# JunyiPeng00/wespeaker_hubert

Measured on AMD Instinct MI355X. Metric: embeddings/sec on 5s 16kHz utts, higher is better.
Workload: dtype f32 (bf16x3 split MFMA, fp32 accumulate)

## Files before the change

wespeaker_hubert_amd/csrc/astp_fused.h:

```cpp
#pragma once

#include "common.h"

namespace wsp {

struct AstpArgs {
  const float* att;
  const float* x;
  int ldx, B, T, C;
  const int* seg;
  const void* w2;
  const float* bias2;
  float var_floor;
  float* out;
};
bool astp_fused_supported(int C, int K);
void launch_astp_fused(const AstpArgs& p, hipStream_t s);

}
```

wespeaker_hubert_amd/csrc/astp_fused.hip:

```cpp
#include "astp_fused.h"
#include "gemm_common.h"

namespace wsp {

namespace {

typedef __bf16 bf16x8 __attribute__((ext_vector_type(8)));

constexpr int kK = 128;

typedef __attribute__((address_space(3))) void lds_void;

__device__ __forceinline__ void dma16(__amdgpu_buffer_rsrc_t r, unsigned char* lds, int voff) {
  __builtin_amdgcn_raw_ptr_buffer_load_lds(r, (lds_void*)lds, 16, voff, 0, 0, 0);
}

constexpr int kCB2 = 256;
constexpr int kChunkBytes = 32 * kK * 4;

constexpr int kLds3 = 3 * kChunkBytes;

__global__ __launch_bounds__(512, 1) void astp_fused3_kernel(const AstpArgs p) {
  extern __shared__ __attribute__((aligned(16))) unsigned char ring[];
  const int tid = threadIdx.x;
  const int lane = tid & 63;
  const int wave = tid >> 6;
  const int r32 = lane & 31;
  const int h = lane >> 5;
  const int nct = p.C / kCB2;
  const int id = xcd_remap(blockIdx.x, gridDim.x);
  const int b = id / nct;
  const int ct = id - b * nct;
  const int r0 = p.seg ? p.seg[b] : b * p.T;
  const int T = p.seg ? p.seg[b + 1] - r0 : p.T;
  const int col = ct * kCB2 + wave * 32 + r32;
  const __amdgpu_buffer_rsrc_t ra = make_rsrc(p.att + (size_t)r0 * kK);
  const __amdgpu_buffer_rsrc_t rx = make_rsrc(p.x + (size_t)r0 * p.ldx);

  auto dma_chunk = [&](int t0, int slot) {
#pragma unroll
    for (int j = 0; j < 2; ++j) {
      const int piece = 2 * wave + j;
      const int row = 2 * piece + h;
      const int c = r32 ^ (row & 15);
      const int t = t0 + row;
      dma16(ra, ring + slot * kChunkBytes + piece * 1024, t < T ? (t * kK + c * 4) * 4 : kOOB);
    }
  };
  auto load_x = [&](int t0, float (&xv)[16]) {
#pragma unroll
    for (int r = 0; r < 16; ++r) {
      const int t = t0 + (r & 3) + 8 * (r >> 2) + 4 * h;
      xv[r] = __builtin_bit_cast(float, __builtin_amdgcn_raw_buffer_load_b32(
                                            rx, t < T ? (t * p.ldx + col) * 4 : kOOB, 0, 0));
    }
  };
  bf16x8 wf[16];
  {
    const __amdgpu_buffer_rsrc_t rw = make_rsrc(p.w2);
    const int ntile = p.C / 32;
#pragma unroll
    for (int i = 0; i < 16; ++i)
      wf[i] = __builtin_bit_cast(bf16x8, __builtin_amdgcn_raw_buffer_load_b128(
                                             rw, ((i * ntile + ct * (kCB2 / 32) + wave) * 64 + lane) * 16, 0, 0));
  }
  const float bias = p.bias2[col];

  float m = -INFINITY, s = 0.f, a1 = 0.f, a2 = 0.f;
  auto consume = [&](int t0, int slot, const float (&xv)[16]) {
    const unsigned char* ab = ring + slot * kChunkBytes + r32 * 512;
    f32x16 acc;
#pragma unroll
    for (int r = 0; r < 16; ++r) acc[r] = 0.f;
#pragma unroll
    for (int ks = 0; ks < 8; ++ks) {
      const int c0 = 4 * ks + 2 * h;
      const f32x4 v0 = *reinterpret_cast<const f32x4*>(ab + ((c0 ^ (r32 & 15)) << 4));
      const f32x4 v1 = *reinterpret_cast<const f32x4*>(ab + (((c0 + 1) ^ (r32 & 15)) << 4));
      bf16x8 ah, al;
#pragma unroll
      for (int e = 0; e < 8; ++e) {
        const float v = e < 4 ? v0[e] : v1[e - 4];
        const __bf16 hh = (__bf16)v;
        ah[e] = hh;
        al[e] = (__bf16)(v - (float)hh);
      }
      acc = __builtin_amdgcn_mfma_f32_32x32x16_bf16(al, wf[2 * ks], acc, 0, 0, 0);
      acc = __builtin_amdgcn_mfma_f32_32x32x16_bf16(ah, wf[2 * ks + 1], acc, 0, 0, 0);
      acc = __builtin_amdgcn_mfma_f32_32x32x16_bf16(ah, wf[2 * ks], acc, 0, 0, 0);
    }
    float ev[16], mc = -INFINITY;
#pragma unroll
    for (int r = 0; r < 16; ++r) {
      const int t = t0 + (r & 3) + 8 * (r >> 2) + 4 * h;
      ev[r] = t < T ? acc[r] + bias : -INFINITY;
      mc = fmaxf(mc, ev[r]);
    }
    if (mc != -INFINITY) {
      const float m1 = fmaxf(m, mc);
      const float sc = __expf(m - m1);
      s *= sc;
      a1 *= sc;
      a2 *= sc;
#pragma unroll
      for (int r = 0; r < 16; ++r) {
        const float pe = __expf(ev[r] - m1);
        s += pe;
        a1 = fmaf(pe, xv[r], a1);
        a2 = fmaf(pe * xv[r], xv[r], a2);
      }
      m = m1;
    }
  };

  float xa[16], xb[16], xc[16];
  const int nch = (T + 31) / 32;
  dma_chunk(0, 0);
  load_x(0, xa);
  if (nch > 1) {
    dma_chunk(32, 1);
    load_x(32, xb);
  }
  auto step = [&](int c, int slot, const float (&xcur)[16], float (&xnext2)[16]) {
    if (c + 1 < nch)
      asm volatile("s_waitcnt vmcnt(18)" ::: "memory");
    else
      asm volatile("s_waitcnt vmcnt(0)" ::: "memory");
    __syncthreads();
    if (c + 2 < nch) {
      dma_chunk((c + 2) * 32, slot == 0 ? 2 : slot - 1);
      load_x((c + 2) * 32, xnext2);
    }
    consume(c * 32, slot, xcur);
  };
  for (int c = 0; c < nch; c += 3) {
    step(c, 0, xa, xc);
    if (c + 1 >= nch) break;
    step(c + 1, 1, xb, xa);
    if (c + 2 >= nch) break;
    step(c + 2, 2, xc, xb);
  }
  const float mo = __shfl_xor(m, 32), so = __shfl_xor(s, 32), a1o = __shfl_xor(a1, 32), a2o = __shfl_xor(a2, 32);
  const float M = fmaxf(m, mo);
  const float f0 = m == -INFINITY ? 0.f : __expf(m - M);
  const float f1 = mo == -INFINITY ? 0.f : __expf(mo - M);
  const float S = s * f0 + so * f1;
  const float A1 = a1 * f0 + a1o * f1;
  const float A2 = a2 * f0 + a2o * f1;
  if (h == 0) {
    const float mean = A1 / S;
    p.out[(size_t)b * 2 * p.C + col] = mean;
    p.out[(size_t)b * 2 * p.C + p.C + col] = sqrtf(fmaxf(A2 / S - mean * mean, p.var_floor));
  }
}

}

bool astp_fused_supported(int C, int K) { return K == kK && C > 0 && C % kCB2 == 0; }

void launch_astp_fused(const AstpArgs& p, hipStream_t s) {
  WSP_CHECK(astp_fused_supported(p.C, kK) && p.B > 0 && (p.seg || p.T > 0), "astp_fused: bad shape");
  WSP_CHECK(p.seg || (long long)p.T * p.ldx * 4 < (long long)kOOB, "astp_fused: utterance exceeds 2 GiB");
  hipLaunchKernelGGL(astp_fused3_kernel, dim3(p.B * (p.C / kCB2)), dim3(512), kLds3, s, p);
  WSP_HIP(hipGetLastError());
}

}
```

wespeaker_hubert_amd/csrc/conv_gemm.hip:

```cpp
#include "gemm_common.h"

namespace wsp {

namespace {

constexpr int BK = 32;
constexpr int LDK = BK + 4;

template <int WM, int WN, int TM, int TN, int AMODE, bool UNI>
__global__ __launch_bounds__(256, 2) void conv_gemm_f32(const ConvGemmArgs p) {
  constexpr int BM = WM * TM * 32;
  constexpr int BN = WN * TN * 32;
  constexpr int AR = BM / 32;
  constexpr int BR = BN / 32;
  static_assert(WM * WN == 4, "4 waves");

  extern __shared__ __attribute__((aligned(16))) float smem[];
  float* As = smem;
  float* Bs = smem + 2 * BM * LDK;

  const int tid = threadIdx.x;
  const int lane = tid & 63;
  const int wave = tid >> 6;
  const int ntiles = p.N / BN;
// ... 31 lines not shown
#pragma unroll
    for (int i = 0; i < BR; ++i)
      *reinterpret_cast<f32x4*>(b + (srow + 32 * i) * LDK + c4) = rb[i];
  };

  const int wm = wave / WN;
  const int wn = wave - wm * WN;
  const int r32 = lane & 31;
  const int h = lane >> 5;

  f32x16 acc[TM][TN];
#pragma unroll
  for (int i = 0; i < TM; ++i)
#pragma unroll
    for (int j = 0; j < TN; ++j)
#pragma unroll
      for (int r = 0; r < 16; ++r) acc[i][j][r] = 0.f;

  const int nk = p.Kp / BK;
  load_tile(0);
  store_tile(0);
  __syncthreads();

  for (int kt = 0; kt < nk; ++kt) {
    const int cur = kt & 1;
    if (kt + 1 < nk) load_tile((kt + 1) * BK);
    const float* a = As + cur * BM * LDK + (wm * TM * 32 + r32) * LDK + h * 16;
    const float* b = Bs + cur * BN * LDK + (wn * TN * 32 + r32) * LDK + h * 16;
#pragma unroll
    for (int q = 0; q < 4; ++q) {
      f32x4 af[TM], bf[TN];
#pragma unroll
      for (int i = 0; i < TM; ++i) af[i] = *reinterpret_cast<const f32x4*>(a + i * 32 * LDK + q * 4);
#pragma unroll
      for (int j = 0; j < TN; ++j) bf[j] = *reinterpret_cast<const f32x4*>(b + j * 32 * LDK + q * 4);
#pragma unroll
      for (int s = 0; s < 4; ++s)
#pragma unroll
        for (int i = 0; i < TM; ++i)
#pragma unroll
          for (int j = 0; j < TN; ++j)
            acc[i][j] = __builtin_amdgcn_mfma_f32_32x32x2f32(af[i][s], bf[j][s], acc[i][j], 0, 0, 0);
    }
    if (kt + 1 < nk) store_tile(cur ^ 1);
    __syncthreads();
  }

  gemm_epilogue<TM, TN>(p, acc, m0, n0, wm, wn, lane);
}

template <int WM, int WN, int TM, int TN, int AMODE, bool UNI>
void launch_k(const ConvGemmArgs& p, hipStream_t s) {
  constexpr int BM = WM * TM * 32, BN = WN * TN * 32;
  const int nwg = ((p.M + BM - 1) / BM) * (p.N / BN);
  const size_t lds = (size_t)2 * (BM + BN) * LDK * sizeof(float);
  hipLaunchKernelGGL((conv_gemm_f32<WM, WN, TM, TN, AMODE, UNI>), dim3(nwg), dim3(256), lds, s, p);
  WSP_HIP(hipGetLastError());
}

template <int WM, int WN, int TM, int TN>
void launch_tile(const ConvGemmArgs& p, hipStream_t s) {
  const bool uni = uniform_ktiles(p);
  if (p.amode == kAAdd) {
    if (uni) launch_k<WM, WN, TM, TN, kAAdd, true>(p, s);
    else launch_k<WM, WN, TM, TN, kAAdd, false>(p, s);
  } else {
    if (uni) launch_k<WM, WN, TM, TN, kACat, true>(p, s);
    else launch_k<WM, WN, TM, TN, kACat, false>(p, s);
  }
}

}

int conv_gemm_tile_for(int N) { return (N % 128 == 0) ? 0 : 1; }

void launch_conv_gemm(const ConvGemmArgs& args, hipStream_t s) {
  const ConvGemmArgs p = normalized(args);
  check_conv_args(p, "conv_gemm");
  WSP_CHECK(!p.colsum, "conv_gemm: column sums are a bf16x3-kernel epilogue");
  WSP_CHECK(!p.conv2d && p.N % 64 == 0, "conv_gemm (f32): 1-D convs with N % 64 == 0 only");
  WSP_CHECK(!p.gcols || p.gcols % 64 == 0, "conv_gemm (f32): grouped columns must be a multiple of 64");
  WSP_CHECK(!p.sc2d && !p.lnmode && !p.gate,
            "conv_gemm (f32): conv3 + shortcut, the LayerNorm fold and the gated A tail run on tile family 7");
  if (conv_gemm_tile_for(p.N) == 0 && !p.gcols)
    launch_tile<2, 2, 2, 2>(p, s);
  else
    launch_tile<4, 1, 1, 2>(p, s);
}

}
```

wespeaker_hubert_amd/csrc/conv_gemm_x3.hip:

```cpp
#include "conv_gemm_x3_impl.h"

namespace wsp {

int conv_gemm_x3_block_rows(const ConvGemmArgs& p, int variant) {
  if (p.N % 64 != 0 || (p.gcols && p.gcols % 64 != 0)) return 128;
  if (p.gcols || p.N % 128 != 0) return 128;
  return variant == 3 ? 128 : 256;
}

namespace {
__global__ __launch_bounds__(256) void colsum_mean_kernel(const double* __restrict__ part, int bm, int T, int N,
                                                          float* __restrict__ out, int ldo) {
  const int b = blockIdx.y;
  const int n = blockIdx.x * 256 + threadIdx.x;
  if (n >= N) return;
  const long r0 = (long)b * T, r1 = r0 + T;
  double v = 0.0;
  for (long mt = r0 / bm; mt * bm < r1; ++mt) {
    const int slot = (mt * bm) / T == b ? 0 : 1;
    v += part[((size_t)mt * 2 + slot) * N + n];
  }
  out[(long)b * ldo + n] = (float)(v / (double)T);
}
}

void launch_colsum_mean(const double* part, int block_rows, int T, int B, int N, float* out, int ldo,
                        hipStream_t s) {
  WSP_CHECK(block_rows > 0 && T >= block_rows && B > 0 && N > 0, "colsum_mean: bad shape");
  hipLaunchKernelGGL(colsum_mean_kernel, dim3((N + 255) / 256, B), dim3(256), 0, s, part, block_rows, T, N, out,
                     ldo);
  WSP_HIP(hipGetLastError());
}

bool conv_gemm_x3_gate_ok(const ConvGemmArgs& args, int variant) {
  return variant == 7 && args.gate && x3::g256_gate_supported(normalized(args));
}

void launch_conv_gemm_x3(const ConvGemmArgs& args, const void* whi, const void* wlo, int variant,
                         hipStream_t s) {
  const ConvGemmArgs p = normalized(args);
  check_conv_args(p, "conv_gemm_x3");
  if (p.colsum) {
    const int bm = conv_gemm_x3_block_rows(p, variant);
    WSP_CHECK(!p.seg && !p.row_bias && !p.conv2d && p.T >= bm,
              "conv_gemm_x3: column sums need a uniform batch with T >= block rows and no row bias");
  }
  WSP_CHECK(p.Kp % 64 == 0, "conv_gemm_x3: packed K must be a multiple of 64");
  WSP_CHECK(variant >= 3 && variant <= 7, "conv_gemm_x3: tile family must be 3, 4, 5, 6 or 7");
  const __bf16* h = static_cast<const __bf16*>(whi);
  const __bf16* l = static_cast<const __bf16*>(wlo);
  x3::TileFn f;
  WSP_CHECK(!p.lnmode || (variant == 7 && x3::g256_supported(p)),
            "conv_gemm_x3: the LayerNorm fold runs on tile family 7 only");
  WSP_CHECK(!p.sc2d || (variant == 7 && x3::g256_supported(p)),
            "conv_gemm_x3: conv3 + shortcut runs on tile family 7 only (N % 256 == 0, 16-B aligned operands)");
  WSP_CHECK(!p.gate || (variant == 7 && x3::g256_gate_supported(p)),
            "conv_gemm_x3: the gated A tail runs on tile family 7 only (conv_gemm_x3_gate_ok)");
  if (variant == 7 && x3::g256_supported(p)) {
    x3::t_g256(p, h, l, s);
    return;
  }
  if (variant == 7) variant = 6;
  if (p.N % 64 != 0 || (p.gcols && p.gcols % 64 != 0)) {
    f = x3::t_4x1_1x1;
  } else if (p.gcols) {
    f = variant >= 5 ? x3::t_8x1_1x2_sw : x3::t_4x1_1x2;
  } else if (p.N % 128 != 0) {
    f = x3::t_4x1_1x2;
  } else if (variant == 3) {
    f = x3::t_2x2_2x2_sw;
  } else if (variant == 4) {
    f = x3::t_4x2_2x2_sw;
  } else if (p.N % 256 == 0) {
    f = variant == 6 ? x3::t_4x2_2x4_mf16 : x3::t_4x2_2x4_sw1;
  } else {
    f = x3::t_4x2_2x2_sw;
  }
  f(p, h, l, s);
}

}
```

wespeaker_hubert_amd/csrc/conv_gemm_x3_impl.h:

```cpp
#pragma once

#include <type_traits>

#include "gemm_common.h"

namespace wsp {

namespace {

typedef __bf16 bf16x8 __attribute__((ext_vector_type(8)));
typedef __bf16 bf16x4 __attribute__((ext_vector_type(4)));

constexpr int BK = 32;

template <bool SWZ, int MF = 32>
struct Lds {
  static constexpr int ROWB = SWZ ? 64 : 80;
  static constexpr int SKEW = SWZ ? 0 : 64;
  __device__ __forceinline__ static int off(int row, int byte) {
    static_assert(MF == 32 || SWZ, "16x16 fragments need the swizzled rows");
    if constexpr (SWZ && MF == 16)
      return row * 64 + ((((byte >> 4) ^ (0x1320 >> (4 * ((row >> 2) & 3)))) & 3) << 4) + (byte & 15);
    else if constexpr (SWZ) return row * 64 + ((((byte >> 4) ^ (row >> 2)) & 3) << 4) + (byte & 15);
    else return row * 80 + byte;
  }
};

template <int WM, int WN, int TM, int TN, int AMODE, bool UNI, int ROLE, bool C2D = false, bool SWZ = false,
          int NSET = 2, int MF = 32>
__global__ __launch_bounds__(WM* WN * 64, 2) void conv_gemm_x3(const ConvGemmArgs p,
                                                               const __bf16* __restrict__ whi,
                                                               const __bf16* __restrict__ wlo) {
  using L = Lds<SWZ, MF>;
  static_assert(MF == 32 || NSET == 1, "16x16 MFMA: one-staging-set wide tiles only");
  constexpr int ROWB = L::ROWB;
  constexpr int NT = WM * WN * 64;
  constexpr int BM = WM * TM * 32;
  constexpr int BN = WN * TN * 32;
  constexpr int AR = BM * 8 / NT;
  constexpr int BR = BN * 8 / NT;
  constexpr int ROWS_A = NT / 8;
  constexpr int A_BYTES = BM * ROWB;
  constexpr int B_BYTES = BN * ROWB;
  constexpr int B_LO = B_BYTES + L::SKEW;
  constexpr int STAGE = 2 * A_BYTES + B_LO + B_BYTES;
  static_assert(AR >= 1 && BR >= 1, "tile too small for the thread count");
  static_assert(BN * 4 % 64 == 0, "a W image must be a whole number of wave loads");

  extern __shared__ __attribute__((aligned(16))) unsigned char smem[];

  const int tid = threadIdx.x;
  const int lane = tid & 63;
  const int wave = tid >> 6;
  const int ntiles = p.N / BN;
  const int mtiles = (p.M + BM - 1) / BM;
  const int wg = xcd_remap(blockIdx.x, ntiles * mtiles);
  const int mt = wg / ntiles;
  const int nt = wg - mt * ntiles;
  const int m0 = mt * BM;
  const int n0 = nt * BN;

  const int srow = tid >> 3;
  const int c4 = (tid & 7) * 4;
  std::conditional_t<C2D, ALoader2D<AR>, ALoader<AR, AMODE, UNI>> al;
  al.init(p, m0, srow, ROWS_A, c4);
  if (p.gcols) al.a0 += (n0 / p.gcols) * p.gcin;
  const __amdgpu_buffer_rsrc_t rwhi = make_rsrc(whi);
  const __amdgpu_buffer_rsrc_t rwlo = make_rsrc(wlo);
  int boff[BR], bls[BR];
  bool bimg[BR];
#pragma unroll
  for (int i = 0; i < BR; ++i) {
    const int q = tid + NT * i;
    const int img = __builtin_amdgcn_readfirstlane(q / (BN * 4));
    const int qq = q - img * BN * 4;
    const int row = qq >> 2, part = qq & 3;
    bimg[i] = img != 0;
    boff[i] = ((n0 + row) * p.Kp + part * 8) * 2;
    bls[i] = L::off(row, part * 16) + (img ? B_LO : 0);
  }

  f32x4 ra0[AR], ra1[AR];
  bf16x8 rb0[BR], rb1[BR];

  auto load_tile = [&](f32x4 (&ra)[AR], bf16x8 (&rb)[BR], int k0, bool live) {
#pragma unroll
    for (int i = 0; i < BR; ++i) {
      const int o = live ? boff[i] + k0 * 2 : kOOB;
      rb[i] = __builtin_bit_cast(bf16x8, __builtin_amdgcn_raw_buffer_load_b128(bimg[i] ? rwlo : rwhi, o, 0, 0));
    }
    al.load(k0, ra, live);
  };

  auto store_tile = [&](const f32x4 (&ra)[AR], const bf16x8 (&rb)[BR], int buf) {
    unsigned char* st = smem + buf * STAGE;
#pragma unroll
    for (int i = 0; i < AR; ++i) {
      bf16x4 hi, lo;
#pragma unroll
      for (int e = 0; e < 4; ++e) {
        const float x = ra[i][e];
        const __bf16 hh = (__bf16)x;
        hi[e] = hh;
        lo[e] = (__bf16)(x - (float)hh);
      }
      const int off = L::off(srow + ROWS_A * i, c4 * 2);
      *reinterpret_cast<bf16x4*>(st + off) = hi;
      *reinterpret_cast<bf16x4*>(st + A_BYTES + off) = lo;
    }
// ... 78 lines not shown
        }
    };
    load_tile(ra0, rb0, 0, true);
    store_tile(ra0, rb0, 0);
    load_tile(ra0, rb0, BK, true);
    __syncthreads();
    for (int kt = 0; kt < nk; ++kt) {
      const int buf = kt & 1;
      const unsigned char* st = smem + buf * STAGE;
      rdA(st, 0);
      rdB(st, 0);
      mm(0, 0);
      rdB(st, 1);
      mm(0, 1);
      store_tile(ra0, rb0, buf ^ 1);
      load_tile(ra0, rb0, (kt + 2) * BK, kt + 2 < nk);
      rdA(st, 1);
      mm(1, 1);
      rdB(st, 0);
      mm(1, 0);
      __syncthreads();
    }
    gemm_epilogue16<2 * TM, 2 * TN, WM, WN>(p, acc16, m0, n0, wm, wn, lane, smem);
    return;
  } else if constexpr (NSET == 1) {
    load_tile(ra0, rb0, 0, true);
    store_tile(ra0, rb0, 0);
    load_tile(ra0, rb0, BK, true);
    __syncthreads();
    for (int kt = 0; kt < nk; ++kt) {
      const int buf = kt & 1;
      mma_step(buf, 0);
      store_tile(ra0, rb0, buf ^ 1);
      load_tile(ra0, rb0, (kt + 2) * BK, kt + 2 < nk);
      mma_step(buf, 1);
      __syncthreads();
    }
    gemm_epilogue<TM, TN, WM, WN>(p, acc, m0, n0, wm, wn, lane, smem);
    return;
  }
  load_tile(ra0, rb0, 0, true);
  load_tile(ra1, rb1, BK, true);
  store_tile(ra0, rb0, 0);
  __syncthreads();

  if constexpr (ROLE == 2) {
    for (int kt = 0; kt < nk - 2; kt += 2) {
      load_tile(ra0, rb0, (kt + 2) * BK, true);
      mma_step(0, 0);
      store_tile(ra1, rb1, 1);
      mma_step(0, 1);
      __syncthreads();
      load_tile(ra1, rb1, (kt + 3) * BK, true);
      mma_step(1, 0);
      store_tile(ra0, rb0, 0);
      mma_step(1, 1);
      __syncthreads();
    }
    float rv[TM][TN][16];
    load_residual_tiles<TM, TN>(p, rv, m0, n0, wm, wn, lane);
    mma_step(0, 0);
    store_tile(ra1, rb1, 1);
    mma_step(0, 1);
    __syncthreads();
    mma_step(1, 0);
    mma_step(1, 1);
    gemm_epilogue_res_pre<TM, TN>(p, acc, m0, n0, wm, wn, lane, rv);
    return;
  }

  for (int kt = 0; kt < nk; kt += 2) {
    load_tile(ra0, rb0, (kt + 2) * BK, kt + 2 < nk);
    mma_step(0, 0);
    store_tile(ra1, rb1, 1);
    mma_step(0, 1);
    __syncthreads();
    load_tile(ra1, rb1, (kt + 3) * BK, kt + 3 < nk);
    mma_step(1, 0);
    store_tile(ra0, rb0, 0);
    mma_step(1, 1);
    __syncthreads();
  }

  gemm_epilogue<TM, TN, WM, WN>(p, acc, m0, n0, wm, wn, lane, smem);
}

template <int WM, int WN, int TM, int TN, int AMODE, bool UNI, int ROLE, bool C2D, bool SWZ, int NSET, int MF = 32>
void launch_x3_k(const ConvGemmArgs& p, const __bf16* whi, const __bf16* wlo, hipStream_t s) {
  constexpr int BM = WM * TM * 32, BN = WN * TN * 32, NT = WM * WN * 64;
  constexpr int ROWB = Lds<SWZ>::ROWB;
  const int nwg = ((p.M + BM - 1) / BM) * (p.N / BN);
  const size_t lds = (size_t)2 * (2 * BM * ROWB + 2 * BN * ROWB + Lds<SWZ>::SKEW);
  hipLaunchKernelGGL((conv_gemm_x3<WM, WN, TM, TN, AMODE, UNI, ROLE, C2D, SWZ, NSET, MF>), dim3(nwg), dim3(NT), lds,
                     s, p, whi, wlo);
  WSP_HIP(hipGetLastError());
}

template <int WM, int WN, int TM, int TN, bool SWZ = false, int NSET = 2, int MF = 32>
void launch_x3_tile(const ConvGemmArgs& p, const __bf16* whi, const __bf16* wlo, hipStream_t s) {
  if constexpr (MF == 32) {
    if (p.conv2d) {
      launch_x3_k<WM, WN, TM, TN, kACat, true, 0, true, SWZ, NSET, MF>(p, whi, wlo, s);
      return;
    }
  }
  const bool uni = uniform_ktiles(p);
  if (MF == 32 && p.amode == kAAdd) {
    if constexpr (MF == 32) {
      if (uni)
        launch_x3_k<WM, WN, TM, TN, kAAdd, true, 0, false, SWZ, NSET, MF>(p, whi, wlo, s);
      else
        launch_x3_k<WM, WN, TM, TN, kAAdd, false, 0, false, SWZ, NSET, MF>(p, whi, wlo, s);
    }
  } else if (!uni) {
    launch_x3_k<WM, WN, TM, TN, kACat, false, 0, false, SWZ, NSET, MF>(p, whi, wlo, s);
  } else if (p.role == 1) {
    launch_x3_k<WM, WN, TM, TN, kACat, true, 1, false, SWZ, NSET, MF>(p, whi, wlo, s);
  } else if constexpr (NSET == 2 && TM * TN <= 4) {
    if (p.res && p.role == 2)
      launch_x3_k<WM, WN, TM, TN, kACat, true, 2, false, SWZ, NSET>(p, whi, wlo, s);
    else
      launch_x3_k<WM, WN, TM, TN, kACat, true, 0, false, SWZ, NSET>(p, whi, wlo, s);
  } else {
    launch_x3_k<WM, WN, TM, TN, kACat, true, 0, false, SWZ, NSET, MF>(p, whi, wlo, s);
  }
}

}

namespace x3 {
using TileFn = void (*)(const ConvGemmArgs&, const __bf16*, const __bf16*, hipStream_t);
void t_4x1_1x1(const ConvGemmArgs&, const __bf16*, const __bf16*, hipStream_t);
void t_4x1_1x2(const ConvGemmArgs&, const __bf16*, const __bf16*, hipStream_t);
void t_8x1_1x2_sw(const ConvGemmArgs&, const __bf16*, const __bf16*, hipStream_t);
void t_2x2_2x2_sw(const ConvGemmArgs&, const __bf16*, const __bf16*, hipStream_t);
void t_4x2_2x2_sw(const ConvGemmArgs&, const __bf16*, const __bf16*, hipStream_t);
void t_4x2_2x4_sw1(const ConvGemmArgs&, const __bf16*, const __bf16*, hipStream_t);
void t_4x2_2x4_mf16(const ConvGemmArgs&, const __bf16*, const __bf16*, hipStream_t);
bool g256_supported(const ConvGemmArgs&);
bool g256_gate_supported(const ConvGemmArgs&);
void t_g256(const ConvGemmArgs&, const __bf16*, const __bf16*, hipStream_t);
}

}
```

wespeaker_hubert_amd/csrc/ecapa_model.cpp:

```cpp
#include "astp_fused.h"
#include "model_impl.h"
#include "res2_chain.h"
#include "xi_pool.h"

namespace wsp {

namespace {
struct Ecapa final : Model::Impl {
  using Impl::Impl;
  int C = 512;
  bool glob = false;
  bool xi = false;
  ConvW layer1;
  struct Block {
    ConvW c1, c3, res2[7];
    LinW se1, se2;
    void* r2w = nullptr;
    float *r2b = nullptr, *r2s = nullptr, *r2t = nullptr;
  } blk[3];
  ConvW conv, pool1, pool2;
  ConvW conv_g;
  void* pool2_frag = nullptr;
  LinW pool1_ctx;
  float *prior_mean = nullptr, *prior_logprec = nullptr;
// ... 247 lines not shown
    g.gate_k0 = 2 * C;
    fill(g, wcat, M, T, 1, 0, xp, 1536, kActRelu, nullptr, true, seg, B);
    fold = conv_gemm_x3_gate_ok(g, opt.x3_variant);
    if (fold) gcat = g;
  }

  gemm("layer1", layer1, feats, feat_dim, x[1], C, M, T, 1, 2, kActRelu, s, seg, B);
  for (int li = 0; li < 3; ++li) {
    const Block& b = blk[li];
    const int dil = li + 2;
    const float* xin = x[li + 1];
    gemm("conv1x1_CxC", b.c1, xin, C, h1, C, M, T, 1, 0, kActRelu, s, seg, B, nullptr, true, 1);
    if (opt.precision == 1 && opt.res2_fused && b.r2w) {
      Res2Args r{};
      r.x = h1;
      r.out = h2;
      r.ldx = r.ldo = C;
      r.M = M;
      r.T = T;
      r.dil = dil;
      r.variant = w == 128 ? opt.res2_variant : std::min(opt.res2_variant, 3);
      r.rout = res2_chain_rout(dil, r.variant, M);
      r.seg = seg;
      r.nseg = B;
      r.w = b.r2w;
      r.bias = b.r2b;
      r.scale = b.r2s;
      r.shift = b.r2t;
      run("res2_k3", 7 * 2.0 * M * w * 3 * w, s, [&] { launch_res2_chain(r, w, s); });
    } else {
      for (int i = 0; i < 7; ++i) {
        ConvGemmArgs g{};
        g.amode = i == 0 ? kACat : kAAdd;
        if (i == 0) {
          one_operand(g, h1, C, w);
        } else {
          g.a[0] = h1 + i * w;
          g.a[1] = h2 + (i - 1) * w;
          g.a[2] = h1;
        }
        gemm3("res2_k3", g, b.res2[i], dil, dil, h2 + i * w, C);
      }
    }
    {
      ConvGemmArgs g{};
      g.amode = kACat;
      g.a[0] = h2;
      g.a[1] = h1 + 7 * w;
      g.a[2] = h1;
      g.cseg[1] = 7 * w;
      g.cseg[2] = g.cseg[3] = C;
      g.role = 1;
      if (se_fused) g.colsum = W.sesum;
      gemm3("conv1x1_CxC", g, b.c3, 1, 0, h3, C);
    }
    run("se", 0, s, [&] {
      if (se_fused) launch_colsum_mean(W.sesum, se_bm, T, B, C, W.gmean, C, s);
      else launch_frame_stats(h3, C, B, T, C, W.gmean, C, 0, 0, s, seg);
      launch_small_linear({W.gmean, C, b.se1.wt, b.se1.bias, W.ghid, 128, B, C, 128, 1}, s);
      launch_small_linear({W.ghid, 128, b.se2.wt, b.se2.bias, W.gate, C, B, 128, C, 3}, s);
    });
    if (li == 2 && fold) continue;
    run("se.scale", 0, s, [&] {
      launch_residual_scale(opt.cat_gate && li == 2 ? nullptr : xin, h3, W.gate, x[li + 2], B, T, C, s, seg, M);
    });
  }
  gemm3("conv_cat", gcat, wcat, 1, 0, xp, 1536);
  if (glob) {
    run("glob_ctx", 0, s, [&] {
      launch_frame_stats(xp, 1536, B, T, 1536, W.gstats, 3072, 1, 1536, s, seg);
      launch_small_linear({W.gstats, 3072, pool1_ctx.wt, pool1_ctx.bias, W.rowb, 128, B, 3072, 128, 0}, s);
    });
  }
  if (xi) {
    gemm("xi_lin1", pool1, xp, 1536, W.att, 256, M, T, 1, 0, kActRelu, s, seg, B);
    gemm("xi_lin2", pool2, W.att, 256, W.logit, 1536, M, T, 1, 0, kActNone, s, seg, B);
    const XiPoolArgs a{W.logit, 1536, xp, 1536, prior_mean, prior_logprec, B, T, 1536, seg, W.pooled, 1536};
    run("xi_pool", 0, s, [&] { launch_xi_pool(a, s); });
    run("head", 0, s, [&] {
      launch_small_linear({W.pooled, 1536, head.wt, head.bias, embed, embed_dim, B, 1536, embed_dim, 0}, s);
    });
    return;
  }
  gemm("pool_linear1", pool1, xp, 1536, W.att, 128, M, T, 1, 0, kActTanh, s, seg, B, glob ? W.rowb : nullptr, !glob);
  if (opt.precision == 1 && opt.astp_fused) {
    AstpArgs a{W.att, xp, 1536, B, T, 1536, seg, pool2_frag, pool2.bias, 1e-7f, W.pooled};
    run("astp", 2.0 * M * 1536 * 128, s, [&] { launch_astp_fused(a, s); });
  } else {
    gemm("pool_linear2", pool2, W.att, 128, W.logit, 1536, M, T, 1, 0, kActNone, s, seg, B);
    run("astp", 0, s, [&] { launch_astp_pool(W.logit, xp, B, T, 1536, W.pooled, s, seg); });
  }
  run("head", 0, s, [&] {
    launch_small_linear({W.pooled, 3072, head.wt, head.bias, embed, embed_dim, B, 3072, embed_dim, 0}, s);
  });
}

}
```

wespeaker_hubert_amd/csrc/kernels.h:

```cpp
#pragma once

#include <vector>

#include "common.h"

namespace wsp {

enum AMode { kACat = 0, kAAdd = 1 };
enum Act { kActNone = 0, kActRelu = 1, kActTanh = 2, kActGelu = 3 };

struct ConvGemmArgs {
  const float* a[3];
  int lda[3];
  int cseg[4];
  int cin, taps, dil, pad;
  int M, T, N;
  const float* w;
  int K, Kp;
  const float* bias;
  const float* row_bias;
  const float* res;
  int ldres;
  const float* scale;
  const float* shift;
  float* out;
  int ldo;
  int act;
  int amode;
  int role;
  int conv2d;
  int Fi, Ti, Fo, To, stride, kw;
  int sc2d;
  int gcols, gcin;
  const int* seg;
  const int* iseg;
  int nseg;
  double* colsum;
  int lnmode;
  float* ln_out;
  const float* ln_in;
  int ln_parts;
  const float* ln_cs;
  const float* ln_g;
  const float* ln_b;
  float ln_eps;
  const float* gate;
  int ldg, gate_k0;
};

inline ConvGemmArgs normalized(ConvGemmArgs p) {
  if (!p.conv2d && !p.sc2d) {
    if (p.stride <= 0) p.stride = 1;
    if (p.Ti <= 0) p.Ti = p.T;
  }
  return p;
}

int conv_gemm_x3_block_rows(const ConvGemmArgs& p, int variant);
void launch_colsum_mean(const double* part, int block_rows, int T, int B, int N, float* out, int ldo,
                        hipStream_t s);
void launch_conv_gemm_x3(const ConvGemmArgs& p, const void* whi, const void* wlo, int variant,
                         hipStream_t s);
bool conv_gemm_x3_gate_ok(const ConvGemmArgs& p, int variant);


void launch_conv_gemm(const ConvGemmArgs& p, hipStream_t s);
int conv_gemm_tile_for(int N);

struct SmallLinearArgs {
  const float* in;
  int ldin;
  const float* wt;
  const float* bias;
  float* out;
  int ldo;
  int R, K, N;
  int act;
  float* scratch = nullptr;
  size_t scratch_floats = 0;
};
void launch_small_linear(const SmallLinearArgs& p, hipStream_t s);
size_t small_linear_scratch_floats(int R, int N, int K);


void launch_frame_stats(const float* x, int ldx, int B, int T, int C, float* out, int ldo,
                        int with_std, int std_off, hipStream_t s, const int* seg = nullptr);

void launch_residual_scale(const float* x, const float* h, const float* g, float* out, int B,
                           int T, int C, hipStream_t s, const int* seg = nullptr, int M = 0);

void launch_astp_pool(const float* e, const float* x, int B, int T, int C, float* out,
                      hipStream_t s, const int* seg = nullptr, float var_floor = 1e-7f);

int simam_chunks(int B, int rows);
void launch_simam(const float* z, const float* res, float* out, int B, int rows, int C, double* part, float* coef,
                  hipStream_t s);
void launch_nhwc_to_tfc(const float* in, float* out, int B, int F, int T, int C, hipStream_t s);

void launch_resnet_stem(const float* feats, int B, int T, int F, int C0, const float* w, const float* bias,
                        float* out, hipStream_t s);

struct FbankConfig {
  int num_bins = 80, sample_rate = 16000, window = 0;
  double frame_length_ms = 25.0, frame_shift_ms = 10.0, low_freq = 20.0, high_freq = 0.0;
  int frame_len = 0, frame_shift = 0, padded = 0;
};
void fbank_config_resolve(FbankConfig& c);
void fbank_mel_banks(const FbankConfig& c, std::vector<float>& w);
struct FbankPlan {
  FbankConfig cfg;
  bool fixed = false;
  int len0 = 0, len1 = 0;
  std::vector<double> host_tab;
  const double* tab = nullptr;
};
void fbank_plan(const FbankConfig& c, FbankPlan& p);
void launch_fbank(const void* wav, int dtype, int B, int N, int ld, float scale, float* feats,
                  int T, int cmn, const FbankPlan& plan, hipStream_t s, const int* wseg = nullptr,
                  const int* fseg = nullptr);

void launch_hubert_conv0(const float* wav, int B, int N, int ldw, int T0, const float* w, const float* gamma,
                         const float* beta, double* stats, float* out, hipStream_t s, const int* wseg = nullptr,
                         const int* oseg = nullptr);
size_t hubert_conv0_stats_doubles(int B, int T0);
void launch_hubert_pos_conv(const float* x, int ldx, const int* seg, int B, int maxT, int M, const void* whi,
                            const void* wlo, int ldw, int gout, const float* bias, float* out, int ldo,
                            hipStream_t s);
struct LayerNormArgs {
  const float* x;
  int ldx;
// ... 42 lines not shown
```

wespeaker_hubert_amd/csrc/model.cpp:

```cpp
#include "model_impl.h"

namespace wsp {

int detail::chunk_for(int B, size_t bytes) {
  const int bc = std::min((int)std::max<size_t>(1, kOperandCap / bytes), B);
  const int chunks = (B + bc - 1) / bc;
  return (B + chunks - 1) / chunks;
}

void Model::Impl::add(const std::string& n, std::vector<int64_t> shape) {
  idx[n] = (int)params.size();
  params.push_back(Param{n, std::move(shape), {}, false});
}
void Model::Impl::add_bn(const std::string& p, int64_t c) {
  add(p + ".weight", {c});
  add(p + ".bias", {c});
  add(p + ".running_mean", {c});
  add(p + ".running_var", {c});
  add(p + ".num_batches_tracked", {});
}
const std::vector<float>& Model::Impl::P(const std::string& n) const {
  auto it = idx.find(n);
  WSP_CHECK(it != idx.end(), "missing parameter " + n);
  const Param& p = params[it->second];
// ... 189 lines not shown
  const int ns = impl->nsub(B);
  size_t bytes = 256;
  for (int i = 0; i < ns; ++i) bytes += impl->ws_bytes_one(B * (i + 1) / ns - B * i / ns, T);
  return bytes;
}

void Model::forward(const float* feats, int B, int T, float* embed, void* ws, size_t ws_bytes,
                    hipStream_t s) {
  Impl& m = *impl;
  WSP_CHECK(!m.is_frontend(), "HuBERT handle: use the front-end forward");
  WSP_CHECK(m.finalized, "forward before finalize");
  if (m.min_frames() >= 2)
    WSP_CHECK(B > 0 && T > 1, "forward needs B >= 1 and T >= 2 frames");
  else
    WSP_CHECK(B > 0 && T >= 1, "forward needs B >= 1 and T >= 1 frames");
  WSP_CHECK((size_t)B * T < (1u << 31), "B*T too large");
  WSP_CHECK(ws_bytes >= workspace_bytes(B, T), "workspace too small");
  m.check_forward(B, T);
  char* wsb = reinterpret_cast<char*>((reinterpret_cast<uintptr_t>(ws) + 255) & ~uintptr_t(255));
  const int ns = m.nsub(B);
  if (ns > 1) m.fork(s, ns);
  for (int i = 0; i < ns; ++i) {
    const int b0 = B * i / ns, nb = B * (i + 1) / ns - b0;
    const float* f = feats + (size_t)b0 * T * m.feat_dim;
    float* e = embed + (size_t)b0 * m.embed_dim;
    m.forward(f, nb, T, e, reinterpret_cast<float*>(wsb), m.sub(s, i));
    wsb += m.ws_bytes_one(nb, T);
  }
  if (ns > 1) m.join(s, ns);
}

size_t Model::workspace_bytes_segments(int B, int M) const {
  WSP_CHECK(impl->has_segments(), "segmented batches are implemented for ECAPA-TDNN handles");
  WSP_CHECK(B > 0 && M >= B, "segmented batch needs B >= 1 and M >= B rows");
  return impl->ws_floats_segments(B, M) * sizeof(float) + 256;
}

void Model::forward_segments(const float* feats, int B, const int* seg, int M, float* embed, void* ws,
                             size_t ws_bytes, hipStream_t s) {
  Impl& m = *impl;
  WSP_CHECK(m.has_segments(), "segmented batches are implemented for ECAPA-TDNN handles");
  WSP_CHECK(m.finalized, "forward before finalize");
  WSP_CHECK(seg != nullptr && B > 0 && M >= B, "segmented batch needs offsets, B >= 1 and M >= B rows");
  WSP_CHECK((size_t)M * 1536 < (1u << 31) / 4, "segmented batch too large");
  WSP_CHECK(ws_bytes >= workspace_bytes_segments(B, M), "workspace too small");
  float* wsf = reinterpret_cast<float*>((reinterpret_cast<uintptr_t>(ws) + 255) & ~uintptr_t(255));
  m.forward_segments(feats, B, seg, M, embed, wsf, s);
}

void Model::profile(bool on) {
  if (on && !impl->prof)
    for (auto& kv : impl->prof_map) {
      kv.second.used = 0;
      kv.second.flops = 0;
    }
  impl->prof = on;
}

namespace {
struct Opt {
  const char* key;
  int Options::*field;
  int lo, hi, hole;
  const char* err;
};
using I = Options;
constexpr int kNoHole = -1000;
const Opt kOpts[] = {
    {"precision", &I::precision, 0, 1, kNoHole, "precision must be 0 (f32) or 1 (bf16x3)"},
    {"streams", &I::streams, 1, 8, kNoHole, "streams must be 1..8"},
    {"layer", &I::layer, -1, 12, kNoHole, "layer must be -1 (weighted sum) or 0..12"},
    {"in_planes", &I::in_planes, 32, 64, kNoHole, "in_planes must be 32 or 64"},
    {"res2_fused", &I::res2_fused, 0, 1, kNoHole, "res2_fused must be 0 or 1"},
    {"cam_fused", &I::cam_fused, 0, 1, kNoHole, "cam_fused must be 0 (separate BN-ReLU pass) or 1 (GEMM prologue)"},
    {"ib_fused", &I::ib_fused, 0, 1, kNoHole, "ib_fused must be 0 (conv1, depthwise conv, conv3) or 1 (conv1, fused tail)"},
    {"cat_gate", &I::cat_gate, 0, 1, kNoHole, "cat_gate must be 0 or 1"},
    {"gate_fold", &I::gate_fold, 0, 1, kNoHole, "gate_fold must be 0 or 1"},
    {"res_prefetch", &I::res_prefetch, 0, 1, kNoHole, "res_prefetch must be 0 or 1"},
    {"res_tail", &I::res_tail, 0, 2, kNoHole, "res_tail must be 0 (off), 1 (tail + next conv1) or 2 (tail alone)"},
    {"sc_fuse", &I::sc_fuse, 0, 3, kNoHole, "sc_fuse must be 0 .. 3 (bit 0: one GEMM, bit 1: in the tail)"},
    {"c1_stage_fuse", &I::c1_stage_fuse, 0, 1, kNoHole, "c1_stage_fuse must be 0 or 1"},
    {"astp_fused", &I::astp_fused, 0, 3, kNoHole,
     "astp_fused must be 0 (linear2 GEMM + pooling kernel) or 1 (fused)"},
    {"attn_pipe", &I::attn_pipe, 0, 1, kNoHole, "attn_pipe must be 0 or 1"},
    {"pos_conv", &I::pos_conv, 0, 1, kNoHole,
     "pos_conv must be 0 (grouped implicit GEMM) or 1 (direct grouped conv)"},
    {"ln_fold", &I::ln_fold, 0, 1, kNoHole, "ln_fold must be 0 (LayerNorm kernels) or 1 (folded into the GEMMs)"},
    {"tail_batch", &I::tail_batch, 0, 1, kNoHole,
     "tail_batch must be 0 (CNN layers 4-6 per chunk) or 1 (batch-wide)"},
    {"res2_variant", &I::res2_variant, 0, 4, 1,
     "res2_variant must be 0 (4 waves, 2 x 2), 2 (4 waves on N, 4 W k-steps in flight), 3 (8 waves) "
     "or 4 (halo-free strips, c1024 widths; else as 3)"},
    {"x3_variant", &I::x3_variant, 0, 9, kNoHole,
     "x3_variant must be 3, 4, 5, 6 (5 on 16x16x32 MFMAs) or 7 (6 staged by LDS-DMA)"},
    {"conv3x3_img", &I::conv3x3_img, 0, 3, kNoHole,
     "conv3x3_img must be 0 (off), 1 (32 / 64 channels) or 2 / 3 (also 128)"},
};
const Opt& find_opt(const std::string& key) {
  for (const Opt& o : kOpts)
    if (key == o.key) return o;
  throw InvalidArg{"unknown option " + key};
}
}

void Model::set_option(const std::string& key, int value) {
  Impl& m = *impl;
  if (key == "attn_lds" || key == "conv1x1_rows") return;
  const Opt& o = find_opt(key);
  if (key == "layer") {
    WSP_CHECK(m.owns_option(key), "option 'layer' applies to the HuBERT front end");
    WSP_CHECK(!m.finalized, "option 'layer' must be set before finalize");
  } else if (key == "in_planes") {
    WSP_CHECK(m.owns_option(key), "option 'in_planes' applies to SimAM-ResNet handles");
    WSP_CHECK(!m.finalized, "option 'in_planes' must be set before finalize");
    WSP_CHECK(value == 32 || value == 64, o.err);
    for (const auto& p : m.params) WSP_CHECK(!p.set, "option 'in_planes' must be set before the weights");
  }
  WSP_CHECK(value >= o.lo && value <= o.hi && value != o.hole, o.err);
  if (key == "x3_variant") {
    value = value >= 3 && value <= 7 ? value : value == 8 ? 7 : 5;
  } else if (key == "astp_fused") {
    value = value ? 1 : 0;
  }
  m.opt.*o.field = value;
  if (key == "in_planes") m.build_params();
}

int Model::get_option(const std::string& key) const { return impl->opt.*find_opt(key).field; }

void Model::profile_query(const std::string& tag, int* launches, double* total_ms, double* flops) {
  *launches = 0;
  *total_ms = 0;
  *flops = 0;
  double fl = 0;
  for (auto& kv : impl->prof_map) {
    const std::string& k = kv.first;
    if (k != tag && k.compare(0, tag.size() + 1, tag + ".") != 0) continue;
    ProfEntry& e = kv.second;
    for (size_t i = 0; i < e.used; ++i) {
      WSP_HIP(hipEventSynchronize(e.ev[i].second));
      float ms = 0;
      WSP_HIP(hipEventElapsedTime(&ms, e.ev[i].first, e.ev[i].second));
      *total_ms += ms;
    }
    *launches += (int)e.used;
    fl += e.flops;
  }
  *flops = *launches ? fl / (double)*launches : 0.0;
}

}
```

wespeaker_hubert_amd/csrc/model_impl.h:

```cpp
#pragma once

#include <hip/hip_runtime.h>

#include <cmath>
#include <cstdint>
#include <algorithm>
#include <map>
#include <string>
#include <vector>

#include "kernels.h"
#include "model.h"
#include "pack.h"

namespace wsp {

namespace detail {

constexpr double kBnEps = 1e-5;

struct DevBuf {
  std::vector<void*> ptrs;
  ~DevBuf() {
    for (void* p : ptrs) (void)hipFree(p);
  }
  template <typename T>
  T* upload(const std::vector<T>& v) {
    void* p = nullptr;
    WSP_HIP(hipMalloc(&p, std::max<size_t>(v.size(), 1) * sizeof(T)));
    ptrs.push_back(p);
    if (!v.empty()) WSP_HIP(hipMemcpy(p, v.data(), v.size() * sizeof(T), hipMemcpyHostToDevice));
    return static_cast<T*>(p);
  }
  void* upload_u16(const std::vector<uint16_t>& v) { return upload(v); }
};

struct ConvW {
  float* w = nullptr;
  void* whi = nullptr;
  void* wlo = nullptr;
  float* bias = nullptr;
  float* scale = nullptr;
  float* shift = nullptr;
  int N = 0, cin = 0, taps = 1, K = 0, Kp = 0;
  void* frag = nullptr;
};

struct LinW {
  float* wt = nullptr;
  float* bias = nullptr;
  int K = 0, N = 0;
};

inline int round_up(int a, int b) { return (a + b - 1) / b * b; }

constexpr size_t kOperandCap = ((size_t)1 << 31) / 8 * 7;
int chunk_for(int B, size_t bytes);

struct WsCursor {
  float* base = nullptr;
  size_t off = 0;
  static size_t padded(size_t n) { return (n + 63) / 64 * 64; }
  float* take(size_t n) {
    float* p = base ? base + off : nullptr;
    off += padded(n);
    return p;
  }
};

}

using namespace detail;

struct Param {
  std::string name;
  std::vector<int64_t> shape;
  std::vector<float> host;
  bool set = false;
  int64_t numel() const {
    int64_t n = 1;
    for (auto s : shape) n *= s;
    return n;
  }
};

struct ProfEntry {
  std::vector<std::pair<hipEvent_t, hipEvent_t>> ev;
  size_t used = 0;
  double flops = 0;
};

struct Options {
  int precision = 1;
  int x3_variant = 5;
  int streams = 1;
  int res2_fused = 1;
  int res2_variant = 4;
  int cat_gate = 1;
  int gate_fold = 1;
  int astp_fused = 1;
  int in_planes = 32;
  int conv3x3_img = 2;
  int res_prefetch = 1;
  int res_tail = 1;
  int sc_fuse = 3;
  int c1_stage_fuse = 1;
  int layer = -1;
  int attn_pipe = 1;
  int pos_conv = 1;
  int ln_fold = 0;
  int tail_batch = 1;
  int cam_fused = 1;
  int ib_fused = 0;
};

struct Model::Impl {
  std::string arch;
  int feat_dim = 80, embed_dim = 192;
  bool emb_bn = false, two_emb = false;
  Options opt;
  std::vector<Param> params;
  std::map<std::string, int> idx;
  bool finalized = false;
  int device = 0;
  DevBuf dev;

  Impl(const std::string& arch, int feat_dim, int embed_dim, bool emb_bn, bool two_emb)
      : arch(arch), feat_dim(feat_dim), embed_dim(embed_dim), emb_bn(emb_bn), two_emb(two_emb) {}
  virtual ~Impl();

  virtual void build_params() = 0;
  virtual void finalize() = 0;
  virtual bool owns_option(const std::string&) const { return false; }
  virtual bool is_frontend() const { return false; }
  virtual void check_forward(int B, int T) const {}
  virtual int min_frames() const { return 2; }
  virtual size_t ws_floats(int B, int T) const = 0;
  virtual void forward(const float* feats, int B, int T, float* embed, float* ws, hipStream_t s) = 0;
  virtual bool has_segments() const { return false; }
  virtual size_t ws_floats_segments(int B, int M) const { return 0; }
  virtual void forward_segments(const float* feats, int B, const int* seg, int M, float* embed, float* ws,
                                hipStream_t s) {}

  std::vector<hipStream_t> sub_st;
  std::vector<hipEvent_t> sub_ev;
  int nsub(int B) const { return std::max(1, std::min(opt.streams, B)); }
  size_t ws_bytes_one(int B, int T) const { return (ws_floats(B, T) * sizeof(float) + 255) & ~size_t(255); }
  hipStream_t sub(hipStream_t s, int i) const { return i == 0 ? s : sub_st[i - 1]; }
  void fork(hipStream_t s, int ns);
  void join(hipStream_t s, int ns);

  void add(const std::string& n, std::vector<int64_t> shape);
  void add_bn(const std::string& p, int64_t c);
  const std::vector<float>& P(const std::string& n) const;
  void bn_affine(const std::string& p, std::vector<double>& sc, std::vector<double>& sh) const;
  struct Folded {
    std::vector<float> w, b;
  };
  Folded fold_bn(const std::string& wname, const std::string& bn) const;

  ConvW pack_conv(const std::vector<float>& w, int N, int cin, int taps, const float* bias, const std::string& bn);
  void* pack_frag(const std::vector<float>& w, int N, int K, pack::FragOrder order = pack::kPlain, int kacc = -1) {
    return dev.upload_u16(pack::frag(w, N, K, order, kacc));
  }
  void* pack_frag_acc(const std::vector<float>& w, int N, int K, int kacc = -1) { return pack_frag(w, N, K, pack::kAcc, kacc); }
  LinW pack_lin(const float* w, int N, int K, int ldk, const float* bias);

  static void one_operand(ConvGemmArgs& g, const float* a, int lda, int cin);
  void fill(ConvGemmArgs& g, const ConvW& cw, int M, int T, int dil, int pad, float* out, int ldo, int act,
            const float* row_bias, bool use_bias, const int* seg, int nseg);
  void launch(const ConvGemmArgs& g, const ConvW& cw, hipStream_t s);
  void gemm(const char* tag, const ConvW& cw, const float* a0, int lda, float* out, int ldo, int M, int T, int dil,
            int pad, int act, hipStream_t s, const int* seg, int nseg, const float* row_bias = nullptr,
            bool use_bias = true, int role = 0);

  bool prof = false;
  std::map<std::string, ProfEntry> prof_map;
  template <typename F>
  void run(const char* tag, double flops, hipStream_t s, F&& f) {
    if (!prof) {
      f();
      return;
    }
// ... 20 lines not shown
```

Measured before the change: 26290.

## Emit pre-split bf16 hi/lo attention planes from pool_linear1 epilogue for fused ASTP

The pool_linear1 tanh GEMM gets a new epilogue that writes its output already split into bf16 high and low halves, staged through LDS and permuted so each 16-byte group holds the hi or lo plane. The fused ASTP kernel then reinterprets the loaded words directly as bf16x8 operands instead of splitting fp32 values into hi/lo bf16 per element inside its MFMA loop. This moves the split arithmetic out of the ASTP inner loop into the producer GEMM epilogue, where each element is split once. It forces the linear1 GEMM onto the 256x128 tile, adds an LDS staging pass with permutes in the epilogue, and is enabled by default via the new astp_split option.

```diff
diff --git a/wespeaker_hubert_amd/csrc/astp_fused.h b/wespeaker_hubert_amd/csrc/astp_fused.h
--- a/wespeaker_hubert_amd/csrc/astp_fused.h
+++ b/wespeaker_hubert_amd/csrc/astp_fused.h
@@ -13,6 +13,7 @@
   const float* bias2;
   float var_floor;
   float* out;
+  int split = 0;
 };
 bool astp_fused_supported(int C, int K);
 void launch_astp_fused(const AstpArgs& p, hipStream_t s);
diff --git a/wespeaker_hubert_amd/csrc/astp_fused.hip b/wespeaker_hubert_amd/csrc/astp_fused.hip
--- a/wespeaker_hubert_amd/csrc/astp_fused.hip
+++ b/wespeaker_hubert_amd/csrc/astp_fused.hip
@@ -20,6 +20,7 @@
 
 constexpr int kLds3 = 3 * kChunkBytes;
 
+template <bool SPLIT>
 __global__ __launch_bounds__(512, 1) void astp_fused3_kernel(const AstpArgs p) {
   extern __shared__ __attribute__((aligned(16))) unsigned char ring[];
   const int tid = threadIdx.x;
@@ -78,12 +79,17 @@
       const f32x4 v0 = *reinterpret_cast<const f32x4*>(ab + ((c0 ^ (r32 & 15)) << 4));
       const f32x4 v1 = *reinterpret_cast<const f32x4*>(ab + (((c0 + 1) ^ (r32 & 15)) << 4));
       bf16x8 ah, al;
+      if constexpr (SPLIT) {
+        ah = __builtin_bit_cast(bf16x8, v0);
+        al = __builtin_bit_cast(bf16x8, v1);
+      } else {
 #pragma unroll
-      for (int e = 0; e < 8; ++e) {
-        const float v = e < 4 ? v0[e] : v1[e - 4];
-        const __bf16 hh = (__bf16)v;
-        ah[e] = hh;
-        al[e] = (__bf16)(v - (float)hh);
+        for (int e = 0; e < 8; ++e) {
+          const float v = e < 4 ? v0[e] : v1[e - 4];
+          const __bf16 hh = (__bf16)v;
+          ah[e] = hh;
+          al[e] = (__bf16)(v - (float)hh);
+        }
       }
       acc = __builtin_amdgcn_mfma_f32_32x32x16_bf16(al, wf[2 * ks], acc, 0, 0, 0);
       acc = __builtin_amdgcn_mfma_f32_32x32x16_bf16(ah, wf[2 * ks + 1], acc, 0, 0, 0);
@@ -161,7 +167,10 @@
 void launch_astp_fused(const AstpArgs& p, hipStream_t s) {
   WSP_CHECK(astp_fused_supported(p.C, kK) && p.B > 0 && (p.seg || p.T > 0), "astp_fused: bad shape");
   WSP_CHECK(p.seg || (long long)p.T * p.ldx * 4 < (long long)kOOB, "astp_fused: utterance exceeds 2 GiB");
-  hipLaunchKernelGGL(astp_fused3_kernel, dim3(p.B * (p.C / kCB2)), dim3(512), kLds3, s, p);
+  if (p.split)
+    hipLaunchKernelGGL(astp_fused3_kernel<true>, dim3(p.B * (p.C / kCB2)), dim3(512), kLds3, s, p);
+  else
+    hipLaunchKernelGGL(astp_fused3_kernel<false>, dim3(p.B * (p.C / kCB2)), dim3(512), kLds3, s, p);
   WSP_HIP(hipGetLastError());
 }
 
diff --git a/wespeaker_hubert_amd/csrc/conv_gemm.hip b/wespeaker_hubert_amd/csrc/conv_gemm.hip
--- a/wespeaker_hubert_amd/csrc/conv_gemm.hip
+++ b/wespeaker_hubert_amd/csrc/conv_gemm.hip
@@ -137,6 +137,7 @@
   WSP_CHECK(!p.gcols || p.gcols % 64 == 0, "conv_gemm (f32): grouped columns must be a multiple of 64");
   WSP_CHECK(!p.sc2d && !p.lnmode && !p.gate,
             "conv_gemm (f32): conv3 + shortcut, the LayerNorm fold and the gated A tail run on tile family 7");
+  WSP_CHECK(!p.out_split, "conv_gemm (f32): the pre-split output is a bf16x3-kernel epilogue");
   if (conv_gemm_tile_for(p.N) == 0 && !p.gcols)
     launch_tile<2, 2, 2, 2>(p, s);
   else
diff --git a/wespeaker_hubert_amd/csrc/conv_gemm_x3.hip b/wespeaker_hubert_amd/csrc/conv_gemm_x3.hip
--- a/wespeaker_hubert_amd/csrc/conv_gemm_x3.hip
+++ b/wespeaker_hubert_amd/csrc/conv_gemm_x3.hip
@@ -56,6 +56,14 @@
             "conv_gemm_x3: conv3 + shortcut runs on tile family 7 only (N % 256 == 0, 16-B aligned operands)");
   WSP_CHECK(!p.gate || (variant == 7 && x3::g256_gate_supported(p)),
             "conv_gemm_x3: the gated A tail runs on tile family 7 only (conv_gemm_x3_gate_ok)");
+  if (p.out_split) {
+    WSP_CHECK(p.N % 128 == 0 && p.act == kActTanh && !p.res && !p.colsum && !p.conv2d && !p.gcols && !p.lnmode &&
+                  !p.sc2d && !p.gate && p.amode == kACat && uniform_ktiles(p) && p.ldo % 4 == 0 &&
+                  (reinterpret_cast<uintptr_t>(p.out) & 15) == 0,
+              "conv_gemm_x3: the pre-split output needs a 1-D tanh GEMM with N % 128 == 0 and a 16-B aligned output");
+    x3::t_4x2_2x2_sw(p, h, l, s);
+    return;
+  }
   if (variant == 7 && x3::g256_supported(p)) {
     x3::t_g256(p, h, l, s);
     return;
diff --git a/wespeaker_hubert_amd/csrc/conv_gemm_x3_impl.h b/wespeaker_hubert_amd/csrc/conv_gemm_x3_impl.h
--- a/wespeaker_hubert_amd/csrc/conv_gemm_x3_impl.h
+++ b/wespeaker_hubert_amd/csrc/conv_gemm_x3_impl.h
@@ -25,6 +25,64 @@
     else return row * 80 + byte;
   }
 };
+
+typedef unsigned u32x4 __attribute__((ext_vector_type(4)));
+template <int TM, int TN, bool RB>
+__device__ __forceinline__ void gemm_epilogue_split(const ConvGemmArgs& p, f32x16 (&acc)[TM][TN], int m0, int n0, int wm,
+                                                    int wn, int wave, int lane, unsigned char* smem) {
+  static_assert(TN == 2, "split epilogue: the 256 x 128 tile's 64-column wave tiles");
+  constexpr int CW = 32 * TN, P = 8 * TN, RPI = 64 / P;
+  unsigned* stg = reinterpret_cast<unsigned*>(smem) + wave * 32 * CW;
+  const int r32 = lane & 31, h = lane >> 5;
+  const int q = lane & (P - 1);
+  const unsigned sel = q & 1 ? 0x07060302u : 0x05040100u;
+  const __amdgpu_buffer_rsrc_t ro = make_rsrc(p.out);
+  float bv[TN], sc[TN], sh[TN];
+#pragma unroll
+  for (int j = 0; j < TN; ++j) {
+    const int col = n0 + (wn * TN + j) * 32 + r32;
+    bv[j] = p.bias ? p.bias[col] : 0.f;
+    sc[j] = p.scale ? p.scale[col] : 1.f;
+    sh[j] = p.scale ? p.shift[col] : 0.f;
+  }
+#pragma unroll
+  for (int i = 0; i < TM; ++i) {
+    const int row0 = m0 + (wm * TM + i) * 32;
+#pragma unroll
+    for (int j = 0; j < TN; ++j) {
+      const int col = n0 + (wn * TN + j) * 32 + r32;
+#pragma unroll
+      for (int r = 0; r < 16; ++r) {
+        const int rr = (r & 3) + 8 * (r >> 2) + 4 * h;
+        float y = acc[i][j][r] + bv[j];
+        if constexpr (RB) {
+          const int row = row0 + rr;
+          const int rowc = row < p.M ? row : p.M - 1;
+          const int ub = p.seg ? seg_of(p.seg, p.nseg, rowc) : rowc / p.T;
+          y += p.row_bias[(size_t)ub * p.N + col];
+        }
+        y = tanhf(y);
+        y = y * sc[j] + sh[j];
+        const __bf16 hh = (__bf16)y;
+        const __bf16 ll = (__bf16)(y - (float)hh);
+        stg[rr * CW + j * 32 + r32] =
+            (unsigned)__builtin_bit_cast(unsigned short, hh) | ((unsigned)__builtin_bit_cast(unsigned short, ll) << 16);
+      }
+    }
+    asm volatile("s_waitcnt lgkmcnt(0)" ::: "memory");
+#pragma unroll
+    for (int u = 0; u < 32 / RPI; ++u) {
+      const int rl = RPI * u + lane / P;
+      const int row = row0 + rl;
+      const u32x4 w0 = *reinterpret_cast<const u32x4*>(stg + rl * CW + (q >> 1) * 8);
+      const u32x4 w1 = *reinterpret_cast<const u32x4*>(stg + rl * CW + (q >> 1) * 8 + 4);
+      const u32x4 o{__builtin_amdgcn_perm(w0[1], w0[0], sel), __builtin_amdgcn_perm(w0[3], w0[2], sel),
+                    __builtin_amdgcn_perm(w1[1], w1[0], sel), __builtin_amdgcn_perm(w1[3], w1[2], sel)};
+      __builtin_amdgcn_raw_buffer_store_b128(o, ro, row < p.M ? (row * p.ldo + n0 + wn * CW) * 4 + q * 16 : kOOB, 0, 0);
+    }
+    asm volatile("s_waitcnt lgkmcnt(0)" ::: "memory");
+  }
+}
 
 template <int WM, int WN, int TM, int TN, int AMODE, bool UNI, int ROLE, bool C2D = false, bool SWZ = false,
           int NSET = 2, int MF = 32>
@@ -269,7 +327,13 @@
     __syncthreads();
   }
 
-  gemm_epilogue<TM, TN, WM, WN>(p, acc, m0, n0, wm, wn, lane, smem);
+  if constexpr (ROLE == 3) {
+    static_assert(TN == 2 && WM * WN * 32 * 64 * 4 <= 2 * STAGE, "split epilogue: 64-column wave tiles staged in LDS");
+    if (p.row_bias) gemm_epilogue_split<TM, TN, true>(p, acc, m0, n0, wm, wn, wave, lane, smem);
+    else gemm_epilogue_split<TM, TN, false>(p, acc, m0, n0, wm, wn, wave, lane, smem);
+  } else {
+    gemm_epilogue<TM, TN, WM, WN>(p, acc, m0, n0, wm, wn, lane, smem);
+  }
 }
 
 template <int WM, int WN, int TM, int TN, int AMODE, bool UNI, int ROLE, bool C2D, bool SWZ, int NSET, int MF = 32>
@@ -285,6 +349,13 @@
 
 template <int WM, int WN, int TM, int TN, bool SWZ = false, int NSET = 2, int MF = 32>
 void launch_x3_tile(const ConvGemmArgs& p, const __bf16* whi, const __bf16* wlo, hipStream_t s) {
+  if (p.out_split) {
+    if constexpr (WM == 4 && WN == 2 && TM == 2 && TN == 2 && SWZ && NSET == 2 && MF == 32)
+      launch_x3_k<WM, WN, TM, TN, kACat, true, 3, false, SWZ, NSET>(p, whi, wlo, s);
+    else
+      WSP_CHECK(false, "conv_gemm_x3: the pre-split output runs on the 256 x 128 tile");
+    return;
+  }
   if constexpr (MF == 32) {
     if (p.conv2d) {
       launch_x3_k<WM, WN, TM, TN, kACat, true, 0, true, SWZ, NSET, MF>(p, whi, wlo, s);
diff --git a/wespeaker_hubert_amd/csrc/ecapa_model.cpp b/wespeaker_hubert_amd/csrc/ecapa_model.cpp
--- a/wespeaker_hubert_amd/csrc/ecapa_model.cpp
+++ b/wespeaker_hubert_amd/csrc/ecapa_model.cpp
@@ -353,9 +353,16 @@
     });
     return;
   }
-  gemm("pool_linear1", pool1, xp, 1536, W.att, 128, M, T, 1, 0, kActTanh, s, seg, B, glob ? W.rowb : nullptr, !glob);
+  const bool split = opt.precision == 1 && opt.astp_fused && opt.astp_split;
+  {
+    ConvGemmArgs g{};
+    one_operand(g, xp, 1536, pool1.cin);
+    g.out_split = split;
+    fill(g, pool1, M, T, 1, 0, W.att, 128, kActTanh, glob ? W.rowb : nullptr, !glob, seg, B);
+    run("pool_linear1", 2.0 * M * pool1.N * pool1.K, s, [&] { launch(g, pool1, s); });
+  }
   if (opt.precision == 1 && opt.astp_fused) {
-    AstpArgs a{W.att, xp, 1536, B, T, 1536, seg, pool2_frag, pool2.bias, 1e-7f, W.pooled};
+    AstpArgs a{W.att, xp, 1536, B, T, 1536, seg, pool2_frag, pool2.bias, 1e-7f, W.pooled, split};
     run("astp", 2.0 * M * 1536 * 128, s, [&] { launch_astp_fused(a, s); });
   } else {
     gemm("pool_linear2", pool2, W.att, 128, W.logit, 1536, M, T, 1, 0, kActNone, s, seg, B);
diff --git a/wespeaker_hubert_amd/csrc/kernels.h b/wespeaker_hubert_amd/csrc/kernels.h
--- a/wespeaker_hubert_amd/csrc/kernels.h
+++ b/wespeaker_hubert_amd/csrc/kernels.h
@@ -46,6 +46,7 @@
   float ln_eps;
   const float* gate;
   int ldg, gate_k0;
+  int out_split;
 };
 
 inline ConvGemmArgs normalized(ConvGemmArgs p) {
diff --git a/wespeaker_hubert_amd/csrc/model.cpp b/wespeaker_hubert_amd/csrc/model.cpp
--- a/wespeaker_hubert_amd/csrc/model.cpp
+++ b/wespeaker_hubert_amd/csrc/model.cpp
@@ -295,6 +295,7 @@
     {"c1_stage_fuse", &I::c1_stage_fuse, 0, 1, kNoHole, "c1_stage_fuse must be 0 or 1"},
     {"astp_fused", &I::astp_fused, 0, 3, kNoHole,
      "astp_fused must be 0 (linear2 GEMM + pooling kernel) or 1 (fused)"},
+    {"astp_split", &I::astp_split, 0, 1, kNoHole, "astp_split must be 0 (fp32 att) or 1 (bf16 hi / lo planes)"},
     {"attn_pipe", &I::attn_pipe, 0, 1, kNoHole, "attn_pipe must be 0 or 1"},
     {"pos_conv", &I::pos_conv, 0, 1, kNoHole,
      "pos_conv must be 0 (grouped implicit GEMM) or 1 (direct grouped conv)"},
diff --git a/wespeaker_hubert_amd/csrc/model_impl.h b/wespeaker_hubert_amd/csrc/model_impl.h
--- a/wespeaker_hubert_amd/csrc/model_impl.h
+++ b/wespeaker_hubert_amd/csrc/model_impl.h
@@ -99,6 +99,7 @@
   int cat_gate = 1;
   int gate_fold = 1;
   int astp_fused = 1;
+  int astp_split = 1;
   int in_planes = 32;
   int conv3x3_img = 2;
   int res_prefetch = 1;
```

After: 26370 (median of 4 runs). Within noise of the previous version (+0.3%).
